# uci-cbcl/RP-Net

Hardware: AMD Instinct MI355X
Metric: support/query pairs/sec (fwd+bwd, 1-shot 256x256, T=5) (higher is better)
Workload: dtype f32

## Files before the change

rpnet_amd/csrc/conv_wgrad.hip:

```cpp
#include <algorithm>
#include <stdlib.h>

#include "common.h"

namespace rpnet {

template <int WM, int WN>
__global__ __launch_bounds__(256) void conv_wgrad_kernel(const rpnet_conv_desc d, const float* __restrict__ dy,
                                                          float* __restrict__ partial, const int M, const int Cin,
                                                          const int Cout, const int tiles_n, const int steps_per_split) {
    constexpr int BM = 64 * WM, BN = 64 * WN, BK = 32;
    constexpr int A_F4 = BM / 32, B_F4 = BN / 32;
    constexpr int A_RW = BM / 4, B_RW = BN / 4;
    __shared__ __attribute__((aligned(16))) float smem[BK * BM + BK * BN];
    float* As = smem;
    float* Bs = smem + BK * BM;

    const int t = threadIdx.x;
    const int lane = t & 63, wv = t >> 6;
    const int li = lane & 31, h = lane >> 5;
    const int wm = wv >> 1, wn = wv & 1;
    const int tm = blockIdx.x / tiles_n, tn = blockIdx.x - tm * tiles_n;
    const int cm0 = tm * BM, n0 = tn * BN;
    const int tap = blockIdx.y;
// ... 112 lines not shown
    const int li = lane & 31, h = lane >> 5;
    const int wm = wv >> 1, wn = wv & 1;
    int tile, z;
    if ((ksplit & 7) == 0) {
        const int xcd = blockIdx.x & 7, j = blockIdx.x >> 3;
        z = (j / tiles) * 8 + xcd;
        tile = j - (j / tiles) * tiles;
    } else {
        z = blockIdx.x / tiles;
        tile = blockIdx.x - z * tiles;
    }
    const int tm = tile / tiles_n, tn = tile - tm * tiles_n;
    const int cm0 = tm * BM, n0 = tn * BN;

    const int H = d.H, W = d.W, HW = H * W;
    const int ups = d.upsample;
    const int Hs = H >> ups, Ws = W >> ups;
    const float* src; int Cs, cc;
    if (cm0 < d.C0) { src = d.x0; Cs = d.C0; cc = cm0; } else { src = d.x1; Cs = d.C1; cc = cm0 - d.C0; }

    const int total_steps = (M + BK - 1) / BK;
    const int s_begin = z * steps_per_split;
    const int s_end = min(s_begin + steps_per_split, total_steps);

    const __amdgpu_buffer_rsrc_t rsx = __builtin_amdgcn_make_buffer_rsrc(
        const_cast<float*>(src), (short)0, (int)((size_t)d.N * Hs * Ws * Cs * 4), 0x00020000);
    const __amdgpu_buffer_rsrc_t rsy = __builtin_amdgcn_make_buffer_rsrc(
        const_cast<float*>(dy), (short)0, (int)((size_t)M * Cout * 4), 0x00020000);
    const int cs4 = Cs * 4;
    int qoff[A_IT], kyv[A_IT], c16[A_IT];
#pragma unroll
    for (int i = 0; i < A_IT; ++i) {
        const int e = t + 256 * i;
        const int r = e >> 4;
        const int kyi = r / SJ, j = r - kyi * SJ;
        kyv[i] = kyi - 1;
        qoff[i] = j - 1 + (kyi - 1) * W;
        c16[i] = (e & 15) * 16;
    }
    f32x4 ra[A_IT], rb[2];
    auto load_tile = [&](int st) {
        const int p0 = st * BK;
#pragma unroll
        for (int i = 0; i < A_IT; ++i) {
            const int q = p0 + qoff[i];
            int pix, yq;
            if (POW2) {
                yq = (q >> lw) & (H - 1);
                pix = ups ? (((q >> (lw + lh)) * Hs + (yq >> 1)) * Ws + ((q & (W - 1)) >> 1)) : q;
            } else {
                const int n = q / HW, rem = q - n * HW;
                yq = rem / W;
                const int xq = rem - yq * W;
                pix = (n * Hs + (yq >> ups)) * Ws + (xq >> ups);
            }
            const int yp = yq - kyv[i];
            const bool ok = (unsigned)q < (unsigned)M && (unsigned)yp < (unsigned)H;
            const int voff = ok ? pix * cs4 + c16[i] : (int)0x80000000;
            ra[i] = __builtin_bit_cast(f32x4, __builtin_amdgcn_raw_buffer_load_b128(rsx, voff, cc * 4, 0));
            if (INSCALE) {
                const float sv = d.in_scale[ok ? pix : 0];
                ra[i] *= d.in_scale_mode == 2 ? 1.f - sv : sv;
            }
        }
#pragma unroll
        for (int i = 0; i < 2; ++i) {
            const int e = t + 256 * i;
            rb[i] = __builtin_bit_cast(f32x4, __builtin_amdgcn_raw_buffer_load_b128(rsy, (p0 + (e >> 4)) * Cout * 4 + (e & 15) * 16, n0 * 4, 0));
        }
    };
    auto store_tile = [&](int st) {
        float* As = smem;
        float* Bs = smem + A_SZ;
#pragma unroll
        for (int i = 0; i < A_IT; ++i) {
            const int e = t + 256 * i;
            if (e < 3 * SJ * (BM / 4)) *reinterpret_cast<f32x4*>(&As[e * 4]) = ra[i];
        }
#pragma unroll
        for (int i = 0; i < 2; ++i) {
            const int e = t + 256 * i;
            const int p = st * BK + (e >> 4);
            const int ox = POW2 ? (p & (W - 1)) : (p % W);
            *reinterpret_cast<f32x4*>(&Bs[e * 4]) = rb[i] * (ox >= 1 ? 1.f : 0.f);
            *reinterpret_cast<f32x4*>(&Bs[B_SZ + e * 4]) = rb[i];
            *reinterpret_cast<f32x4*>(&Bs[2 * B_SZ + e * 4]) = rb[i] * (ox <= W - 2 ? 1.f : 0.f);
        }
    };

    f32x16 acc[9];
#pragma unroll
    for (int a = 0; a < 9; ++a)
#pragma unroll
        for (int r = 0; r < 16; ++r) acc[a][r] = 0.f;

    if (s_begin < s_end) {
        load_tile(s_begin);
        store_tile(s_begin);
        __syncthreads();
        const float* ap = smem + wm * 32 + li + h * BM;
        const float* bp = smem + A_SZ + wn * 32 + li + h * BN;
        for (int st = s_begin; st < s_end; ++st) {
            const bool more = st + 1 < s_end;
            if (more) load_tile(st + 1);
#pragma unroll
            for (int kp = 0; kp < BK / 2; ++kp) {
                const float bm = bp[kp * 2 * BN], b0 = bp[B_SZ + kp * 2 * BN], b1 = bp[2 * B_SZ + kp * 2 * BN];
#pragma unroll
                for (int ky = 0; ky < 3; ++ky) {
                    const float am = ap[(ky * SJ + kp * 2) * BM];
                    const float a0 = ap[(ky * SJ + kp * 2 + 1) * BM];
                    const float a1 = ap[(ky * SJ + kp * 2 + 2) * BM];
                    acc[ky * 3 + 0] = __builtin_amdgcn_mfma_f32_32x32x2f32(am, bm, acc[ky * 3 + 0], 0, 0, 0);
                    acc[ky * 3 + 1] = __builtin_amdgcn_mfma_f32_32x32x2f32(a0, b0, acc[ky * 3 + 1], 0, 0, 0);
                    acc[ky * 3 + 2] = __builtin_amdgcn_mfma_f32_32x32x2f32(a1, b1, acc[ky * 3 + 2], 0, 0, 0);
                }
            }
            __syncthreads();
            if (more) store_tile(st + 1);
            __syncthreads();
        }
    }
    if (z >= ksplit) return;
    const int col = n0 + wn * 32 + li;
#pragma unroll
    for (int tap = 0; tap < 9; ++tap) {
        float* out = partial + ((size_t)(z * 9 + tap) * Cin) * Cout;
#pragma unroll
        for (int r = 0; r < 16; ++r) {
            const int row = cm0 + wm * 32 + (r & 3) + 8 * (r >> 2) + 4 * h;
            out[(size_t)row * Cout + col] = acc[tap][r];
        }
    }
}

static int ilog2_exact(int v) {
    int l = 0;
    while ((1 << l) < v) ++l;
    return (1 << l) == v ? l : -1;
}

void wgrad9_plan(int M, int Cin, int Cout, int* ksplit, int* steps_per_split, int target_blocks) {
    const int tiles = (Cin / 64) * (Cout / 64);
    const int total_steps = (M + 31) / 32;
    long ks = tiles >= target_blocks ? 1 : (target_blocks + tiles - 1) / tiles;
    ks = std::min<long>(ks, std::max(1, total_steps / 8));
    if (ks >= 8) ks = (ks / 8) * 8;
    *steps_per_split = (int)((total_steps + ks - 1) / ks);
    int k2 = (total_steps + *steps_per_split - 1) / *steps_per_split;
    if (ks >= 8) k2 = ((k2 + 7) / 8) * 8;
    *ksplit = k2;
}

__global__ __launch_bounds__(256) void wgrad_reduce_kernel(const float* __restrict__ partial, float* __restrict__ dw,
                                                            int ksplit, int taps, int Cin_g, int Cout, int cin_w,
                                                            int off0, int split, int off1, int accumulate,
                                                            const float* __restrict__ sx, const float* __restrict__ sdy,
                                                            const float* __restrict__ sx1 = nullptr, const int c0_rows = 0) {
    __shared__ float tile[9][32][33];
    const int t = threadIdx.x;
    const int ci0 = blockIdx.x * 32, co0 = blockIdx.y * 32;
    const size_t zstride = (size_t)taps * Cin_g * Cout;
    const int tap_lo = gridDim.z > 1 ? blockIdx.z : 0, tap_hi = gridDim.z > 1 ? blockIdx.z + 1 : taps;
    const int rr = t >> 3, c4 = (t & 7) * 4;
    const int cin = ci0 + rr;
    const bool ok = cin < cin_w;
    const int row = ok ? (cin < split ? off0 + cin : off1 + (cin - split)) : 0;
    const float scl = sx ? ((sx1 && row >= c0_rows) ? *sx1 : *sx) * *sdy : 1.f;
    auto sum_tap = [&](int tap) -> f32x4 {
        f32x4 s0 = {0.f, 0.f, 0.f, 0.f}, s1 = s0, s2 = s0, s3 = s0;
        if (ok) {
            const float* p = partial + ((size_t)tap * Cin_g + row) * Cout + co0 + c4;
            int z = 0;
            for (; z + 4 <= ksplit; z += 4) {
                s0 += *reinterpret_cast<const f32x4*>(p + (size_t)z * zstride);
                s1 += *reinterpret_cast<const f32x4*>(p + (size_t)(z + 1) * zstride);
                s2 += *reinterpret_cast<const f32x4*>(p + (size_t)(z + 2) * zstride);
                s3 += *reinterpret_cast<const f32x4*>(p + (size_t)(z + 3) * zstride);
            }
            for (; z < ksplit; ++z) s0 += *reinterpret_cast<const f32x4*>(p + (size_t)z * zstride);
        }
        f32x4 s = (s0 + s1) + (s2 + s3);
        if (sx) s *= scl;
        return s;
    };
    auto put = [&](int tap, const f32x4 s) {
#pragma unroll
        for (int k = 0; k < 4; ++k) tile[tap][rr][c4 + k] = s[k];
    };
    int tap = tap_lo;
    for (; tap + 3 <= tap_hi; tap += 3) {
        const f32x4 a0 = sum_tap(tap), a1 = sum_tap(tap + 1), a2 = sum_tap(tap + 2);
        put(tap, a0); put(tap + 1, a1); put(tap + 2, a2);
    }
    for (; tap < tap_hi; ++tap) put(tap, sum_tap(tap));
    __syncthreads();
    const int ncin = min(32, cin_w - ci0);
    if (gridDim.z > 1) {
        for (int e = t; e < 32 * ncin; e += 256) {
            const int col = e / ncin, c = e - col * ncin;
            float* o = dw + ((size_t)(co0 + col) * cin_w + ci0 + c) * taps + tap_lo;
            *o = accumulate ? *o + tile[tap_lo][c][col] : tile[tap_lo][c][col];
        }
        return;
    }
    const int rowlen = ncin * taps;
    for (int e = t; e < 32 * rowlen; e += 256) {
        const int col = e / rowlen, r = e - col * rowlen;
        const int c = r / taps, tap = r - c * taps;
        float* o = dw + ((size_t)(co0 + col) * cin_w + ci0) * taps + r;
        *o = accumulate ? *o + tile[tap][c][col] : tile[tap][c][col];
    }
}

static dim3 reduce_grid(int cin_w, int Cout, int taps) {
    const int tx = cdiv(cin_w, 32), ty = Cout / 32;
    return dim3(tx, ty, (long)tx * ty >= 256 ? 1 : taps);
}

__global__ __launch_bounds__(256) void pack_weight_kernel(const float* __restrict__ w, float* __restrict__ wp,
                                                           float* __restrict__ wd, int taps, int Cin_g, int Cout,
                                                           int cin_w, int off0, int split, int off1) {
    __shared__ float tile[9][32][33];
    const int t = threadIdx.x;
    const int ci0 = blockIdx.x * 32, co0 = blockIdx.y * 32;
    const int ncin = min(32, cin_w - ci0);
    const int nel = ncin * taps;
    for (int e = t; e < 32 * nel; e += 256) {
        const int col = e / nel, r = e - col * nel;
        const int c = r / taps, tap = r - c * taps;
        tile[tap][c][col] = w[((size_t)(co0 + col) * cin_w + ci0) * taps + r];
    }
    __syncthreads();
    for (int e = t; e < taps * 32 * 32; e += 256) {
        const int cl = e & 31, c = (e >> 5) & 31, tap = e >> 10;
        if (c < ncin) {
            const int cin = ci0 + c;
            const int row = cin < split ? off0 + cin : off1 + (cin - split);
            wp[(((size_t)tap * (Cin_g >> 2) + (row >> 2)) * Cout + co0 + cl) * 4 + (row & 3)] = tile[tap][c][cl];
        }
    }
    if (wd) {
        for (int e = t; e < taps * 32 * 32; e += 256) {
            const int q = e & 3, c = (e >> 2) & 31, cq = (e >> 7) & 7, tap = e >> 10;
            if (c < ncin) {
                const int cin = ci0 + c;
                const int row = cin < split ? off0 + cin : off1 + (cin - split);
                const int cout = co0 + cq * 4 + q;
                const int tf = taps - 1 - tap;
                wd[(((size_t)tf * (Cout >> 2) + (cout >> 2)) * Cin_g + row) * 4 + q] = tile[tap][c][cq * 4 + q];
            }
        }
    }
}

static void wgrad_plan(int M, int Cin, int Cout, int taps, int* bm, int* bn, int* ksplit, int* steps_per_split) {
    *bm = (Cin % 128 == 0 && taps > 1) ? 128 : 64;
    *bn = (Cout % 128 == 0) ? 128 : 64;
    long tiles = (long)(Cin / *bm) * (Cout / *bn) * taps;
    if (tiles < 1) tiles = 1;
    const int total_steps = (M + 31) / 32;
    int ks = (int)((768 + tiles - 1) / tiles);
    ks = max(1, min(ks, max(1, total_steps / 8)));
    if (taps == 1) ks = min(ks, kWgrad1MaxSplits);
    *steps_per_split = (total_steps + ks - 1) / ks;
    if (taps == 9) *steps_per_split += *steps_per_split & 1;
    *ksplit = (total_steps + *steps_per_split - 1) / *steps_per_split;
}

int conv_wgrad9_split(const rpnet_conv_desc* d, const void* dy, float* part9, int M, int Cin, int Cout, int ks9, int sps9,
                      hipStream_t s);
bool conv_wgrad9_dma_one_plane_ok(const rpnet_conv_desc* d, int M, int sps9);
int conv_wgrad9_split_dma(const rpnet_conv_desc* d, const void* dy, float* part9, int M, int Cin, int Cout, int ks9, int sps9,
                          hipStream_t s);
bool conv_wgrad9_ring_ok(const rpnet_conv_desc* d, int M, int sps9);
int conv_wgrad9_ring(const rpnet_conv_desc* d, const void* dy, float* part9, int M, int Cin, int Cout, int ks9, int sps9, hipStream_t s);
void wgrad1_split_plan(int M, int Cin, int Cout, int* ksplit, int* steps_per_split);
int conv_wgrad1_split(const rpnet_conv_desc* d, const void* dy, float* part, int M, int Cin, int Cout, int ks, int sps, hipStream_t s);

}

extern "C" size_t rpnet_conv_wgrad_workspace_bytes(int N, int H, int W, int cin_gathered, int cout, int taps) {
    int bm, bn, ks, sps;
    rpnet::wgrad_plan(N * H * W, cin_gathered, cout, taps, &bm, &bn, &ks, &sps);
    size_t need = (size_t)ks * taps * cin_gathered * cout * sizeof(float);
    if (taps == 9 && cin_gathered % 64 == 0 && cout % 64 == 0) {
        int ks9, sps9;
        rpnet::wgrad9_plan(N * H * W, cin_gathered, cout, &ks9, &sps9, 512);
        need = std::max(need, (size_t)ks9 * 9 * cin_gathered * cout * sizeof(float));
    }
    return need;
}

extern "C" int rpnet_conv_wgrad(const rpnet_conv_desc* d, const float* dy, float* dw, int cin_w, int cin_off0,
                                int cin_split, int cin_off1, void* workspace, size_t workspace_bytes,
                                rpnet_stream_t stream) {
    using namespace rpnet;
    RPNET_REQUIRE(d && d->x0 && workspace && (dy || dw), RPNET_ERR_ARG, "conv_wgrad: null pointer");
    RPNET_REQUIRE((dy && dw) || (d->split_planes && d->dilation <= 1), RPNET_ERR_ARG,
                  "conv_wgrad: the two-phase form (dy or dw NULL) exists for the split kernels only");
    const int Cin = d->C0 + d->C1, Cout = d->Co0 + d->Co1;
    RPNET_REQUIRE(d->taps == 9 || d->taps == 1, RPNET_ERR_ARG, "conv_wgrad: taps must be 9 or 1");
    RPNET_REQUIRE(!d->split_planes || d->dilation <= 1, RPNET_ERR_ARG,
                  "conv_wgrad: split operands are implemented for dense 3x3 and 1x1 taps only");
    RPNET_REQUIRE(Cin % 64 == 0 && Cout % 64 == 0, RPNET_ERR_SHAPE, "conv_wgrad: Cin %d / Cout %d not multiples of 64", Cin, Cout);
    RPNET_REQUIRE((long)d->N * d->H * d->W < (1L << 31), RPNET_ERR_SHAPE, "conv_wgrad: too many pixels");
    const int M = d->N * d->H * d->W;
    RPNET_REQUIRE((size_t)M * (d->C0 > d->C1 ? d->C0 : d->C1) * 4 < (1UL << 31) && (size_t)M * Cout * 4 < (1UL << 31),
                  RPNET_ERR_SHAPE, "conv_wgrad: an operand exceeds the 2 GiB buffer-descriptor range (split the batch)");
    hipStream_t s = (hipStream_t)stream;
    if (d->taps == 9 && d->dilation <= 1) {
        RPNET_REQUIRE(d->C1 == 0 || d->C0 % 64 == 0, RPNET_ERR_SHAPE, "conv_wgrad: source split %d not aligned to 64", d->C0);
        int ks9, sps9;
        wgrad9_plan(M, Cin, Cout, &ks9, &sps9, d->split_planes ? 256 : 512);
        const size_t need9 = (size_t)ks9 * 9 * Cin * Cout * sizeof(float);
        RPNET_REQUIRE(workspace_bytes >= need9, RPNET_ERR_WORKSPACE, "conv_wgrad: workspace %zu < %zu", workspace_bytes, need9);
        const int tiles_n9 = Cout / 64, tiles9 = (Cin / 64) * tiles_n9;
        const int lw = ilog2_exact(d->W), lh = ilog2_exact(d->H);
        float* part9 = (float*)workspace;
        if (d->split_planes) {
            RPNET_REQUIRE(d->split_planes >= 1 && d->split_planes <= 3 && d->in_scale_mode == 0, RPNET_ERR_ARG,
                          "conv_wgrad: split operands take 1 to 3 planes and no in_scale");
            if (dy) {
                const int tv = d->tune & 255;
                const bool dma = (d->split_planes == 2 || conv_wgrad9_dma_one_plane_ok(d, M, sps9)) && tv != 8 && tv != 4;
                const bool ring = dma && tv != 16 && conv_wgrad9_ring_ok(d, M, sps9);
                if (int rc = ring ? conv_wgrad9_ring(d, dy, part9, M, Cin, Cout, ks9, sps9, s)
                             : dma ? conv_wgrad9_split_dma(d, dy, part9, M, Cin, Cout, ks9, sps9, s)
                                   : conv_wgrad9_split(d, dy, part9, M, Cin, Cout, ks9, sps9, s))
                    return rc;
            }
            if (!dw) return RPNET_OK;
            RPNET_REQUIRE(d->split_planes == 3 || (d->acc_scale_x && d->acc_scale_dy), RPNET_ERR_ARG,
                          "conv_wgrad: fp16 planes need acc_scale_x and acc_scale_dy");
            hipLaunchKernelGGL(wgrad_reduce_kernel, reduce_grid(cin_w, Cout, 9), dim3(256), 0, s, part9, dw, ks9, 9, Cin,
                               Cout, cin_w, cin_off0, cin_split, cin_off1, d->accumulate,
                               d->split_planes <= 2 ? d->acc_scale_x : nullptr, d->acc_scale_dy);
            return check_launch("wgrad_reduce");
        }
#define RPNET_W9(P2, IS, LW, LH)                                                                                   \
    hipLaunchKernelGGL((conv_wgrad9_kernel<P2, IS>), dim3(tiles9 * ks9), dim3(256), 0, s, *d, dy, part9, M, Cin, Cout, \
                       tiles9, tiles_n9, ks9, sps9, LW, LH)
        const bool p2 = lw >= 0 && lh >= 0, is = d->in_scale_mode != 0;
        if (p2 && is) RPNET_W9(true, true, lw, lh);
        else if (p2) RPNET_W9(true, false, lw, lh);
        else if (is) RPNET_W9(false, true, 0, 0);
        else RPNET_W9(false, false, 0, 0);
#undef RPNET_W9
        int rc9 = check_launch("conv_wgrad9");
        if (rc9) return rc9;
        hipLaunchKernelGGL(wgrad_reduce_kernel, reduce_grid(cin_w, Cout, 9), dim3(256), 0, s, part9, dw, ks9, 9, Cin,
                           Cout, cin_w, cin_off0, cin_split, cin_off1, d->accumulate, (const float*)nullptr, (const float*)nullptr);
        return check_launch("wgrad_reduce");
    }
    if (d->split_planes && d->taps == 1) {
        RPNET_REQUIRE(d->split_planes >= 1 && d->split_planes <= 3 && d->in_scale_mode == 0 && d->upsample == 0, RPNET_ERR_ARG,
                      "conv_wgrad: split 1x1 operands take 1 to 3 planes, no in_scale, no upsampling");
        RPNET_REQUIRE(d->C1 == 0 || (d->C0 % 64 == 0 && d->x1), RPNET_ERR_SHAPE, "conv_wgrad: source split %d not aligned to 64", d->C0);
        int ks1, sps1;
        wgrad1_split_plan(M, Cin, Cout, &ks1, &sps1);
        const size_t need1 = (size_t)ks1 * Cin * Cout * sizeof(float);
        RPNET_REQUIRE(workspace_bytes >= need1, RPNET_ERR_WORKSPACE, "conv_wgrad: workspace %zu < %zu", workspace_bytes, need1);
        float* part1 = (float*)workspace;
        if (dy)
            if (int rc = conv_wgrad1_split(d, dy, part1, M, Cin, Cout, ks1, sps1, s)) return rc;
        if (!dw) return RPNET_OK;
        RPNET_REQUIRE(d->split_planes == 3 || (d->acc_scale_x && d->acc_scale_dy), RPNET_ERR_ARG,
                      "conv_wgrad: fp16 planes need acc_scale_x and acc_scale_dy");
        hipLaunchKernelGGL(wgrad_reduce_kernel, reduce_grid(cin_w, Cout, 1), dim3(256), 0, s, part1, dw, ks1, 1, Cin, Cout, cin_w,
                           cin_off0, cin_split, cin_off1, d->accumulate, d->split_planes <= 2 ? d->acc_scale_x : nullptr,
                           d->acc_scale_dy, d->split_planes <= 2 ? d->acc_scale_x1 : nullptr, d->C0);
        return check_launch("wgrad_reduce");
    }
    int bm, bn, ks, sps;
    wgrad_plan(M, Cin, Cout, d->taps, &bm, &bn, &ks, &sps);
    RPNET_REQUIRE(d->C1 == 0 || d->C0 % bm == 0, RPNET_ERR_SHAPE, "conv_wgrad: source split %d not aligned to tile %d", d->C0, bm);
    const size_t need = (size_t)ks * d->taps * Cin * Cout * sizeof(float);
    RPNET_REQUIRE(workspace_bytes >= need, RPNET_ERR_WORKSPACE, "conv_wgrad: workspace %zu < %zu", workspace_bytes, need);
    const int tiles_n = Cout / bn, tiles = (Cin / bm) * tiles_n;
    dim3 grid(tiles, d->taps, ks);
    float* part = (float*)workspace;
    if (bm == 128 && bn == 128)
        hipLaunchKernelGGL((conv_wgrad_kernel<2, 2>), grid, dim3(256), 0, s, *d, dy, part, M, Cin, Cout, tiles_n, sps);
    else if (bm == 128)
        hipLaunchKernelGGL((conv_wgrad_kernel<2, 1>), grid, dim3(256), 0, s, *d, dy, part, M, Cin, Cout, tiles_n, sps);
    else if (bn == 128)
        hipLaunchKernelGGL((conv_wgrad_kernel<1, 2>), grid, dim3(256), 0, s, *d, dy, part, M, Cin, Cout, tiles_n, sps);
    else
        hipLaunchKernelGGL((conv_wgrad_kernel<1, 1>), grid, dim3(256), 0, s, *d, dy, part, M, Cin, Cout, tiles_n, sps);
    int rc = check_launch("conv_wgrad");
    if (rc) return rc;
    hipLaunchKernelGGL(wgrad_reduce_kernel, reduce_grid(cin_w, Cout, d->taps), dim3(256), 0, s, part, dw, ks, d->taps,
                       Cin, Cout, cin_w, cin_off0, cin_split, cin_off1, d->accumulate, (const float*)nullptr, (const float*)nullptr);
    return check_launch("wgrad_reduce");
}

extern "C" int rpnet_pack_conv_weight(const float* w, float* wp, float* wd, int cout, int cin, int taps, int cin_off0,
                                      int cin_split, int cin_off1, int cin_pad, rpnet_stream_t stream) {
    using namespace rpnet;
    RPNET_REQUIRE(w && wp, RPNET_ERR_ARG, "pack_conv_weight: null pointer");
    RPNET_REQUIRE(cout > 0 && cout % 32 == 0 && cin_pad % 4 == 0 && (taps == 9 || taps == 1), RPNET_ERR_SHAPE,
                  "pack_conv_weight: cout %d cin_pad %d taps %d", cout, cin_pad, taps);
    RPNET_REQUIRE(cin > 0 && cin_split >= 0 && cin_split <= cin && cin_off0 >= 0 && cin_off1 >= 0, RPNET_ERR_SHAPE,
                  "pack_conv_weight: cin %d cin_split %d cin_off0 %d cin_off1 %d", cin, cin_split, cin_off0, cin_off1);
    RPNET_REQUIRE((long)cin_off0 + cin_split <= cin_pad && (long)cin_off1 + (cin - cin_split) <= cin_pad, RPNET_ERR_SHAPE,
                  "pack_conv_weight: channel ranges exceed cin_pad");
    RPNET_REQUIRE(pack_ranges_disjoint(cin, cin_off0, cin_split, cin_off1), RPNET_ERR_SHAPE, "pack_conv_weight: channel ranges overlap");
    hipLaunchKernelGGL(pack_weight_kernel, dim3(cdiv(cin, 32), cout / 32), dim3(256), 0, (hipStream_t)stream, w, wp, wd,
                       taps, cin_pad, cout, cin, cin_off0, cin_split, cin_off1);
    return check_launch("pack_conv_weight");
}
```

rpnet_amd/csrc/conv_wgrad_up4.hip:

```cpp
#include <type_traits>

#include "common.h"
#include "lds_dma.h"
#include "split_bf16.h"

namespace rpnet {

using s16x4u = __attribute__((ext_vector_type(4))) short;
typedef __attribute__((address_space(3))) s16x4u lds_s16x4u_t;

template <int N, int I = 0, typename F>
__device__ __forceinline__ void static_for_wu(F&& f) {
    if constexpr (I < N) {
        f(std::integral_constant<int, I>{});
        static_for_wu<N, I + 1>(f);
    }
}

template <bool K64>
__global__ __launch_bounds__(256, 1) void conv_wgrad_up4_kernel(const rpnet_conv_desc d, const unsigned short* __restrict__ dy,
                                                                 float* __restrict__ partial, const int Ml, const int Cin, const int Cout,
                                                                 const int tiles, const int tiles_n, const int ksplit,
                                                                 const int steps_per_split, const int lw, const int lh) {
    constexpr int NP = 2, BK = 32, RB = 128;
// ... 112 lines not shown
    const int cbyte = (16 * (g & 1) + 4 * (L & 3)) * 2;
    const int a_off = krow * RB + (((wm ^ ((krow >> 1) & 1)) << 6) | cbyte);
    const unsigned char* const aptr = smem + a_off;
    int b_off[2];
#pragma unroll
    for (int kxl = 0; kxl < 2; ++kxl) {
        const int r = krow + 2 - (px + kxl);
        b_off[kxl] = BOFF + r * RB + (((wn ^ ((r >> 1) & 1)) << 6) | cbyte);
    }
    const int b_zero = BOFF + ZROW * RB + ((wn << 6) | cbyte);
    auto tr = [&](const unsigned char* p) -> s16x4u { return __builtin_amdgcn_ds_read_tr16_b64_v4i16((lds_s16x4u_t*)p); };

    s16x4u afr[2][2][NP][2], bfr[2][2][NP][2];
    constexpr int NSL = K64 ? 2 : 1;
    const unsigned char* bsel[2][2][NSL][2];
    const unsigned char* bconst[2][2][2];
#pragma unroll
    for (int s2 = 0; s2 < 2; ++s2)
#pragma unroll
        for (int kxl = 0; kxl < 2; ++kxl)
#pragma unroll
            for (int e = 0; e < 2; ++e) {
                bconst[s2][kxl][e] = smem + b_off[kxl] + (16 * s2 + 4 * e) * RB;
#pragma unroll
                for (int sl = 0; sl < NSL; ++sl) bsel[s2][kxl][sl][e] = bconst[s2][kxl][e];
            }
    const unsigned char* const bzero = smem + b_zero;
    auto b_addr = [&](auto sc, const int st) {
        constexpr int s = decltype(sc)::value;
#pragma unroll
        for (int sl = 0; sl < NSL; ++sl)
#pragma unroll
            for (int e = 0; e < 2; ++e) {
                const int q = st * PXS + BK * sl + 16 * s + 4 * e + krow;
                const int ox = q & (Wl - 1);
                bsel[s][0][sl][e] = (px != 0 || ox <= Wl - 2) ? bconst[s][0][e] : bzero;
                bsel[s][1][sl][e] = (px == 0 || ox >= 1) ? bconst[s][1][e] : bzero;
            }
    };
    constexpr int NR = NP * 8, NMMA = (K64 ? 2 : nprod<NP>()) * 4;
    static_assert(NR <= 2 * NMMA, "at most two fragment reads behind each MFMA");
    auto read_frag = [&](auto sc, auto kc, auto stagec) {
        constexpr int s = decltype(sc)::value, k = decltype(kc)::value, stage = decltype(stagec)::value;
        constexpr int grp = k / 8, r = (k - grp * 8) >> 1, e = k & 1;
        constexpr int pa = K64 ? grp : NP - 1 - grp, pb = grp;
        if constexpr (r == 0 || r == 3) {
            constexpr int kyl = r == 0 ? 0 : 1;
            constexpr int off = stage * A_STAGE + pa * A_PLANE + (kyl * BK + 16 * s + 4 * e) * RB;
            afr[s][kyl][pa][e] = tr(aptr + off);
        } else {
            constexpr int kxl = r - 1;
            bfr[s][kxl][pb][e] = tr(bsel[s][kxl][K64 ? pb : 0][e] + (stage * B_STAGE + pb * B_PLANE));
        }
    };
    auto frag = [](const s16x4u lo, const s16x4u hi) {
        return __builtin_bit_cast(bf16x8, __builtin_shufflevector(lo, hi, 0, 1, 2, 3, 4, 5, 6, 7));
    };
    auto mma_one = [&](auto sc, auto mc) {
        constexpr int s = decltype(sc)::value, m = decltype(mc)::value;
        constexpr int q = m / 4, tap = m - q * 4, kyl = tap >> 1, kxl = tap & 1;
        constexpr int pa = K64 ? q : prod_a<NP>(q), pb = K64 ? q : prod_b<NP>(q);
        acc[tap] = mma16<NP>(frag(afr[s][kyl][pa][0], afr[s][kyl][pa][1]), frag(bfr[s][kxl][pb][0], bfr[s][kxl][pb][1]), acc[tap]);
    };
    using I0 = std::integral_constant<int, 0>;
    using I1 = std::integral_constant<int, 1>;

    if (s_begin < s_end) {
        auto stc = [&](int st) { return st < s_end ? st : s_end - 1; };
        dma_step(std::integral_constant<int, 0>{}, s_begin);
        dma_step(std::integral_constant<int, 1>{}, stc(s_begin + 1));
        dma_step(std::integral_constant<int, 2>{}, stc(s_begin + 2));
        wait_all_but_one_step();
        __builtin_amdgcn_s_barrier();
        b_addr(I0{}, s_begin);
        static_for_wu<NR>([&](auto kc) { read_frag(I0{}, kc, I0{}); });
        auto step = [&](auto kc4, const int st) {
            constexpr int K = decltype(kc4)::value;
            using SK = std::integral_constant<int, K>;
            using SN = std::integral_constant<int, (K + 1) & 3>;
            using SD = std::integral_constant<int, (K + 3) & 3>;
            const int dst_step = stc(st + 3);
            b_addr(I1{}, st);
            __builtin_amdgcn_sched_barrier(0);
            static_for_wu<NMMA>([&](auto mc) {
                constexpr int m = decltype(mc)::value;
                mma_one(I0{}, mc);
                __builtin_amdgcn_sched_barrier(0);
                read_frag(I1{}, mc, SK{});
                __builtin_amdgcn_sched_barrier(0);
                if constexpr (m < NR - NMMA) {
                    read_frag(I1{}, std::integral_constant<int, NMMA + m>{}, SK{});
                    __builtin_amdgcn_sched_barrier(0);
                }
                if constexpr (m == NMMA / 2 - 1 || m == NMMA - 3) {
                    dma_x(std::integral_constant<int, (m == NMMA / 2 - 1 ? 0 : 1)>{}, SD{}, dst_step);
                    __builtin_amdgcn_sched_barrier(0);
                }
            });
            b_addr(I0{}, st + 1);
            __builtin_amdgcn_sched_barrier(0);
            static_for_wu<NMMA>([&](auto mc) {
                constexpr int m = decltype(mc)::value;
                mma_one(I1{}, mc);
                __builtin_amdgcn_sched_barrier(0);
                read_frag(I0{}, mc, SN{});
                __builtin_amdgcn_sched_barrier(0);
                if constexpr (m < NR - NMMA) {
                    read_frag(I0{}, std::integral_constant<int, NMMA + m>{}, SN{});
                    __builtin_amdgcn_sched_barrier(0);
                }
                if constexpr (m == NMMA / 2 - 1) {
                    dma_y(SD{}, false, dst_step);
                    __builtin_amdgcn_sched_barrier(0);
                }
                if constexpr (m == NMMA - 3) {
                    if (wv == 0) dma_y(SD{}, true, dst_step);
                    __builtin_amdgcn_sched_barrier(0);
                }
            });
            wait_all_but_one_step();
            __builtin_amdgcn_s_barrier();
        };
        for (int st = s_begin; st < s_end; st += 4) {
            step(std::integral_constant<int, 0>{}, st);
            if (st + 1 >= s_end) break;
            step(std::integral_constant<int, 1>{}, st + 1);
            if (st + 2 >= s_end) break;
            step(std::integral_constant<int, 2>{}, st + 2);
            if (st + 3 >= s_end) break;
            step(std::integral_constant<int, 3>{}, st + 3);
        }
        asm volatile("s_waitcnt vmcnt(0)" ::: "memory");
        __builtin_amdgcn_s_barrier();
    }
    if (z >= ksplit) return;
    const int li = lane & 31, h = lane >> 5;
    constexpr int SW = 36;
    float* slab = reinterpret_cast<float*>(smem) + wv * 32 * SW;
#pragma unroll
    for (int tap = 0; tap < 4; ++tap) {
#pragma unroll
        for (int r = 0; r < 16; ++r) slab[((r & 3) + 8 * (r >> 2) + 4 * h) * SW + li] = acc[tap][r];
        __builtin_amdgcn_wave_barrier();
        float* out = partial + ((size_t)((phase * ksplit + z) * 4 + tap) * Cin + cm0 + wm * 32) * Cout + n0 + wn * 32;
#pragma unroll
        for (int q = 0; q < 4; ++q) {
            const int gidx = q * 64 + lane, rr = gidx >> 3, c4 = gidx & 7;
            *reinterpret_cast<f32x4*>(out + (size_t)rr * Cout + c4 * 4) = *reinterpret_cast<const f32x4*>(&slab[rr * SW + c4 * 4]);
        }
        __builtin_amdgcn_wave_barrier();
    }
}

__global__ __launch_bounds__(256) void wgrad_up4_reduce_kernel(const float* __restrict__ partial, float* __restrict__ dw, const int ksplit,
                                                                const int Cin, const int Cout, const int accumulate,
                                                                const float* __restrict__ sx, const float* __restrict__ sdy) {
    __shared__ float tile[9][32][33];
    const int t = threadIdx.x;
    const int ci0 = blockIdx.x * 32, co0 = blockIdx.y * 32;
    const int rr = t >> 3, c4 = (t & 7) * 4;
    const size_t tstride = (size_t)Cin * Cout, zstride = 4 * tstride, pstride = (size_t)ksplit * zstride;
    const float scl = *sx * *sdy;
    f32x4 v[4][4];
#pragma unroll
    for (int ph = 0; ph < 4; ++ph)
#pragma unroll
        for (int sl = 0; sl < 4; ++sl) {
            const float* p = partial + ph * pstride + sl * tstride + (size_t)(ci0 + rr) * Cout + co0 + c4;
            f32x4 s0 = {0.f, 0.f, 0.f, 0.f}, s1 = s0;
            int z = 0;
            for (; z + 2 <= ksplit; z += 2) {
                s0 += *reinterpret_cast<const f32x4*>(p + (size_t)z * zstride);
                s1 += *reinterpret_cast<const f32x4*>(p + (size_t)(z + 1) * zstride);
            }
            if (z < ksplit) s0 += *reinterpret_cast<const f32x4*>(p + (size_t)z * zstride);
            v[ph][sl] = s0 + s1;
        }
#pragma unroll
    for (int ky = 0; ky < 3; ++ky)
#pragma unroll
        for (int kx = 0; kx < 3; ++kx) {
            f32x4 s = {0.f, 0.f, 0.f, 0.f};
#pragma unroll
            for (int ph = 0; ph < 4; ++ph) {
                const int py = ph >> 1, px = ph & 1;
                const int r = py == 0 ? (ky >= 1) : (ky >= 2), c = px == 0 ? (kx >= 1) : (kx >= 2);
                s += v[ph][r * 2 + c];
            }
            s *= scl;
#pragma unroll
            for (int k = 0; k < 4; ++k) tile[ky * 3 + kx][rr][c4 + k] = s[k];
        }
    __syncthreads();
    const int rowlen = 32 * 9;
    for (int e = t; e < 32 * rowlen; e += 256) {
        const int col = e / rowlen, r = e - col * rowlen;
        const int c = r / 9, tap = r - c * 9;
        float* o = dw + ((size_t)(co0 + col) * Cin + ci0) * 9 + r;
        *o = accumulate ? *o + tile[tap][c][col] : tile[tap][c][col];
    }
}

static int ilog2u(int v) {
    int l = 0;
    while ((1 << l) < v) ++l;
    return (1 << l) == v ? l : -1;
}

static void up4_wgrad_plan(int Ml, int Cin, int Cout, int pxs, int* ksplit, int* sps) {
    const int tiles = (Cin / 64) * (Cout / 64) * 4;
    const int total_steps = (Ml + pxs - 1) / pxs;
    long ks = tiles >= 256 ? 1 : (256 + tiles - 1) / tiles;
    ks = std::min<long>(ks, std::max(1, total_steps / 8));
    if (ks >= 8) ks = (ks / 8) * 8;
    *sps = (int)((total_steps + ks - 1) / ks);
    int k2 = (total_steps + *sps - 1) / *sps;
    if (ks >= 8) k2 = ((k2 + 7) / 8) * 8;
    *ksplit = k2;
}

static bool up4_wgrad_ok(const rpnet_conv_desc* d) {
    if (!d || (d->split_planes != 2 && d->split_planes != 1) || d->C1 || d->Co1 || d->x1 || d->H % 2 || d->W % 2) return false;
    const int Hl = d->H / 2, Wl = d->W / 2;
    if (ilog2u(Wl) < 3 || ilog2u(Hl) < 0 || d->C0 % 64 || d->Co0 % 64) return false;
    const size_t lim = (size_t)1 << 31;
    return (size_t)d->N * Hl * Wl * d->C0 * 4 < lim && (size_t)d->N * d->H * d->W * d->Co0 * 4 < lim &&
           ((size_t)d->N * Hl * Wl) % (d->split_planes == 1 ? 64 : 32) == 0;
}

}

extern "C" int rpnet_conv_wgrad_up4_supported(const rpnet_conv_desc* d) { return rpnet::up4_wgrad_ok(d) ? 1 : 0; }

extern "C" size_t rpnet_conv_wgrad_up4_workspace_bytes(int N, int H, int W, int cin, int cout) {
    int ks, sps, ks1, sps1;
    rpnet::up4_wgrad_plan(N * (H / 2) * (W / 2), cin, cout, 32, &ks, &sps);
    rpnet::up4_wgrad_plan(N * (H / 2) * (W / 2), cin, cout, 64, &ks1, &sps1);
    return (size_t)4 * (ks > ks1 ? ks : ks1) * 4 * cin * cout * sizeof(float);
}

extern "C" int rpnet_conv_wgrad_up4(const rpnet_conv_desc* d, const void* dy, float* dw, void* workspace, size_t workspace_bytes,
                                    rpnet_stream_t stream) {
    using namespace rpnet;
    RPNET_REQUIRE(d && d->x0 && workspace && (dy || dw), RPNET_ERR_ARG, "conv_wgrad_up4: null pointer");
    RPNET_REQUIRE(up4_wgrad_ok(d), RPNET_ERR_SHAPE, "conv_wgrad_up4: N=%d H=%d W=%d C0=%d Co0=%d planes=%d do not fit (rpnet_conv_wgrad_up4_supported)",
                  d->N, d->H, d->W, d->C0, d->Co0, d->split_planes);
    const int Hl = d->H / 2, Wl = d->W / 2, Ml = d->N * Hl * Wl, Cin = d->C0, Cout = d->Co0;
    int ks, sps;
    const bool one = d->split_planes == 1;
    up4_wgrad_plan(Ml, Cin, Cout, one ? 64 : 32, &ks, &sps);
    RPNET_REQUIRE(workspace_bytes >= rpnet_conv_wgrad_up4_workspace_bytes(d->N, d->H, d->W, Cin, Cout), RPNET_ERR_WORKSPACE, "conv_wgrad_up4: workspace");
    hipStream_t s = (hipStream_t)stream;
    float* part = (float*)workspace;
    if (dy) {
        const int tiles_n = Cout / 64, tiles = (Cin / 64) * tiles_n;
        if (one)
            hipLaunchKernelGGL(conv_wgrad_up4_kernel<true>, dim3(tiles * ks * 4), dim3(256), 0, s, *d, (const unsigned short*)dy, part, Ml, Cin, Cout,
                               tiles, tiles_n, ks, sps, ilog2u(Wl), ilog2u(Hl));
        else
            hipLaunchKernelGGL(conv_wgrad_up4_kernel<false>, dim3(tiles * ks * 4), dim3(256), 0, s, *d, (const unsigned short*)dy, part, Ml, Cin, Cout,
                               tiles, tiles_n, ks, sps, ilog2u(Wl), ilog2u(Hl));
        if (int rc = check_launch("conv_wgrad_up4")) return rc;
    }
    if (!dw) return RPNET_OK;
    RPNET_REQUIRE(d->acc_scale_x && d->acc_scale_dy, RPNET_ERR_ARG, "conv_wgrad_up4: fp16 planes need acc_scale_x and acc_scale_dy");
    hipLaunchKernelGGL(wgrad_up4_reduce_kernel, dim3(Cin / 32, Cout / 32), dim3(256), 0, s, (const float*)part, dw, ks, Cin, Cout, d->accumulate,
                       d->acc_scale_x, d->acc_scale_dy);
    return check_launch("wgrad_up4_reduce");
}
```

Measured before the change: 510.4.

## Split wgrad split-K reductions across waves with fewer channels per block

```diff
diff --git a/include/rpnet_wgrad_reduce_abi.h b/include/rpnet_wgrad_reduce_abi.h
--- /dev/null
+++ b/include/rpnet_wgrad_reduce_abi.h
@@ -0,0 +1,18 @@
+#ifndef RPNET_WGRAD_REDUCE_ABI_H
+#define RPNET_WGRAD_REDUCE_ABI_H
+
+#ifdef __cplusplus
+extern "C" {
+#endif
+
+int rpnet_wgrad_reduce(const float* partial, float* dw, int ksplit, int taps, int cin_g, int cout, int cin_w, int cin_off0,
+                       int cin_split, int cin_off1, int accumulate, const float* sx, const float* sdy, const float* sx1,
+                       int c0_rows, void* stream);
+
+int rpnet_wgrad_up4_reduce(const float* partial, float* dw, int ksplit, int cin, int cout, int accumulate, const float* sx,
+                           const float* sdy, void* stream);
+
+#ifdef __cplusplus
+}
+#endif
+#endif
diff --git a/rpnet_amd/csrc/conv_wgrad.hip b/rpnet_amd/csrc/conv_wgrad.hip
--- a/rpnet_amd/csrc/conv_wgrad.hip
+++ b/rpnet_amd/csrc/conv_wgrad.hip
@@ -288,70 +288,122 @@
     *ksplit = k2;
 }
 
-__global__ __launch_bounds__(256) void wgrad_reduce_kernel(const float* __restrict__ partial, float* __restrict__ dw,
-                                                            int ksplit, int taps, int Cin_g, int Cout, int cin_w,
-                                                            int off0, int split, int off1, int accumulate,
-                                                            const float* __restrict__ sx, const float* __restrict__ sdy,
-                                                            const float* __restrict__ sx1 = nullptr, const int c0_rows = 0) {
-    __shared__ float tile[9][32][33];
+
+template <int NT, int ZB>
+__device__ __forceinline__ void reduce_walk(const float* __restrict__ p, const unsigned voff, const size_t tstride, const size_t stride,
+                                            const int count, f32x4 (&s)[NT]) {
+    int k = 0;
+    for (; k + ZB <= count; k += ZB, p += ZB * stride) {
+        f32x4 v[ZB][NT];
+#pragma unroll
+        for (int b = 0; b < ZB; ++b)
+#pragma unroll
+            for (int j = 0; j < NT; ++j) v[b][j] = *reinterpret_cast<const f32x4*>(p + b * stride + j * tstride + voff);
+#pragma unroll
+        for (int b = 0; b < ZB; ++b)
+#pragma unroll
+            for (int j = 0; j < NT; ++j) s[j] += v[b][j];
+    }
+    for (; k < count; ++k, p += stride)
+#pragma unroll
+        for (int j = 0; j < NT; ++j) s[j] += *reinterpret_cast<const f32x4*>(p + j * tstride + voff);
+}
+
+template <int NT, int ZB>
+__device__ __forceinline__ void reduce_chain(const float* __restrict__ p, const unsigned voff, const size_t tstride, const size_t zstride,
+                                             const int q, const int ksplit, f32x4 (&s)[NT]) {
+    const int n = ksplit >> 2;
+#pragma unroll
+    for (int j = 0; j < NT; ++j) s[j] = f32x4{0.f, 0.f, 0.f, 0.f};
+    reduce_walk<NT, ZB>(p + q * zstride, voff, tstride, 4 * zstride, n, s);
+    if (q == 0) reduce_walk<NT, ZB>(p + (size_t)(4 * n) * zstride, voff, tstride, zstride, ksplit - 4 * n, s);
+}
+
+template <int ZC, int TPB>
+__global__ __launch_bounds__(256) __attribute__((amdgpu_waves_per_eu(TPB == 9 ? 4 : 8, 8))) void wgrad_reduce_kernel(
+    const float* __restrict__ partial, float* __restrict__ dw, const int ksplit, const int taps, const int Cin_g, const int Cout,
+    const int cin_w, const int off0, const int split, const int off1, const int accumulate, const float* __restrict__ sx,
+    const float* __restrict__ sdy, const float* __restrict__ sx1, const int c0_rows) {
+#pragma clang fp contract(off)
+    RPNET_PASS_PRIORITY();
+    static_assert(ZC == 1 || ZC == 4, "chains per thread: all four or one");
+    constexpr int CT = 32 / ZC;
+    constexpr int NT = TPB % 3 == 0 ? 3 : 1;
+    constexpr int ZB = NT == 3 ? 2 : 8;
+    constexpr int QS = CT * TPB * 33;
+    __shared__ float tile[ZC * QS];
+    __shared__ float rscl[CT];
     const int t = threadIdx.x;
-    const int ci0 = blockIdx.x * 32, co0 = blockIdx.y * 32;
-    const size_t zstride = (size_t)taps * Cin_g * Cout;
-    const int tap_lo = gridDim.z > 1 ? blockIdx.z : 0, tap_hi = gridDim.z > 1 ? blockIdx.z + 1 : taps;
-    const int rr = t >> 3, c4 = (t & 7) * 4;
-    const int cin = ci0 + rr;
-    const bool ok = cin < cin_w;
-    const int row = ok ? (cin < split ? off0 + cin : off1 + (cin - split)) : 0;
-    const float scl = sx ? ((sx1 && row >= c0_rows) ? *sx1 : *sx) * *sdy : 1.f;
-    auto sum_tap = [&](int tap) -> f32x4 {
-        f32x4 s0 = {0.f, 0.f, 0.f, 0.f}, s1 = s0, s2 = s0, s3 = s0;
-        if (ok) {
-            const float* p = partial + ((size_t)tap * Cin_g + row) * Cout + co0 + c4;
-            int z = 0;
-            for (; z + 4 <= ksplit; z += 4) {
-                s0 += *reinterpret_cast<const f32x4*>(p + (size_t)z * zstride);
-                s1 += *reinterpret_cast<const f32x4*>(p + (size_t)(z + 1) * zstride);
-                s2 += *reinterpret_cast<const f32x4*>(p + (size_t)(z + 2) * zstride);
-                s3 += *reinterpret_cast<const f32x4*>(p + (size_t)(z + 3) * zstride);
-            }
-            for (; z < ksplit; ++z) s0 += *reinterpret_cast<const f32x4*>(p + (size_t)z * zstride);
-        }
-        f32x4 s = (s0 + s1) + (s2 + s3);
-        if (sx) s *= scl;
-        return s;
+    const int ci0 = blockIdx.x * CT, co0 = blockIdx.y * 32, tap0 = blockIdx.z * TPB;
+    const int q = ZC == 4 ? uni(t >> 6) : 0, rr = (t >> 3) & (CT - 1), c4 = (t & 7) * 4;
+    auto gathered = [&](const int cin) { return cin < split ? off0 + cin : off1 + (cin - split); };
+    if (t < CT && ci0 + t < cin_w) rscl[t] = sx ? ((sx1 && gathered(ci0 + t) >= c0_rows) ? *sx1 : *sx) * *sdy : 1.f;
+    if (ci0 + rr < cin_w) {
+        const size_t tstride = (size_t)Cin_g * Cout, zstride = (size_t)taps * tstride;
+        const float* p = partial + (size_t)tap0 * tstride;
+        const unsigned voff = (unsigned)gathered(ci0 + rr) * Cout + co0 + c4;
+        float* lt = tile + (q * CT + rr) * TPB * 33 + c4;
+        const f32x4 zero = {0.f, 0.f, 0.f, 0.f};
+#pragma unroll 1
+        for (int tg = 0; tg < TPB; tg += NT) {
+            f32x4 s[NT];
+            reduce_chain<NT, ZB>(p + tg * tstride, voff, tstride, zstride, q, ksplit, s);
+#pragma unroll
+            for (int j = 0; j < NT; ++j) {
+                if (ZC == 1) s[j] = (s[j] + zero) + (zero + zero);
+#pragma unroll
+                for (int k = 0; k < 4; ++k) lt[(tg + j) * 33 + k] = s[j][k];
+            }
+        }
+    }
+    __syncthreads();
+    const int ncin = min(CT, cin_w - ci0);
+    auto emit = [&](const int rowlen) {
+#pragma unroll 1
+        for (int e = t; e < 32 * rowlen; e += 256) {
+            const int col = e / rowlen, r = e - col * rowlen;
+            const int c = r / TPB;
+            const float* l = tile + r * 33 + col;
+            float v = ZC == 4 ? (l[0] + l[QS]) + (l[2 * QS] + l[3 * QS]) : l[0];
+            v *= rscl[c];
+            float* o = dw + ((size_t)(co0 + col) * cin_w + ci0 + c) * taps + tap0 + (r - c * TPB);
+            *o = accumulate ? *o + v : v;
+        }
     };
-    auto put = [&](int tap, const f32x4 s) {
-#pragma unroll
-        for (int k = 0; k < 4; ++k) tile[tap][rr][c4 + k] = s[k];
-    };
-    int tap = tap_lo;
-    for (; tap + 3 <= tap_hi; tap += 3) {
-        const f32x4 a0 = sum_tap(tap), a1 = sum_tap(tap + 1), a2 = sum_tap(tap + 2);
-        put(tap, a0); put(tap + 1, a1); put(tap + 2, a2);
-    }
-    for (; tap < tap_hi; ++tap) put(tap, sum_tap(tap));
-    __syncthreads();
-    const int ncin = min(32, cin_w - ci0);
-    if (gridDim.z > 1) {
-        for (int e = t; e < 32 * ncin; e += 256) {
-            const int col = e / ncin, c = e - col * ncin;
-            float* o = dw + ((size_t)(co0 + col) * cin_w + ci0 + c) * taps + tap_lo;
-            *o = accumulate ? *o + tile[tap_lo][c][col] : tile[tap_lo][c][col];
-        }
-        return;
-    }
-    const int rowlen = ncin * taps;
-    for (int e = t; e < 32 * rowlen; e += 256) {
-        const int col = e / rowlen, r = e - col * rowlen;
-        const int c = r / taps, tap = r - c * taps;
-        float* o = dw + ((size_t)(co0 + col) * cin_w + ci0) * taps + r;
-        *o = accumulate ? *o + tile[tap][c][col] : tile[tap][c][col];
-    }
-}
-
-static dim3 reduce_grid(int cin_w, int Cout, int taps) {
-    const int tx = cdiv(cin_w, 32), ty = Cout / 32;
-    return dim3(tx, ty, (long)tx * ty >= 256 ? 1 : taps);
+    if (ncin == CT) emit(CT * TPB);
+    else emit(ncin * TPB);
+}
+
+struct ReduceCut { int zc, tpb; };
+static ReduceCut wgrad_reduce_cut(int cin_w, int Cout, int taps, int ksplit) {
+    ReduceCut c;
+    c.zc = ksplit >= 4 ? 4 : 1;
+    c.tpb = 1;
+    if (taps == 9) {
+        const long tiles = (long)cdiv(cin_w, 32 / c.zc) * (Cout / 32);
+        c.tpb = tiles >= 768 ? 9 : 3 * tiles >= 768 ? 3 : 1;
+    }
+    return c;
+}
+
+int launch_wgrad_reduce(const float* partial, float* dw, int ksplit, int taps, int Cin_g, int Cout, int cin_w, int off0, int split,
+                        int off1, int accumulate, const float* sx, const float* sdy, const float* sx1, int c0_rows, hipStream_t s) {
+    const ReduceCut c = wgrad_reduce_cut(cin_w, Cout, taps, ksplit);
+    const dim3 grid(cdiv(cin_w, 32 / c.zc), Cout / 32, taps / c.tpb);
+#define RPNET_RED(ZC, TPB)                                                                                                     \
+    hipLaunchKernelGGL((wgrad_reduce_kernel<ZC, TPB>), grid, dim3(256), 0, s, partial, dw, ksplit, taps, Cin_g, Cout, cin_w, off0, \
+                       split, off1, accumulate, sx, sdy, sx1, c0_rows)
+    if (c.zc == 4) {
+        if (c.tpb == 9) RPNET_RED(4, 9);
+        else if (c.tpb == 3) RPNET_RED(4, 3);
+        else RPNET_RED(4, 1);
+    } else {
+        if (c.tpb == 9) RPNET_RED(1, 9);
+        else if (c.tpb == 3) RPNET_RED(1, 3);
+        else RPNET_RED(1, 1);
+    }
+#undef RPNET_RED
+    return check_launch("wgrad_reduce");
 }
 
 __global__ __launch_bounds__(256) void pack_weight_kernel(const float* __restrict__ w, float* __restrict__ wp,
@@ -469,10 +521,8 @@
             if (!dw) return RPNET_OK;
             RPNET_REQUIRE(d->split_planes == 3 || (d->acc_scale_x && d->acc_scale_dy), RPNET_ERR_ARG,
                           "conv_wgrad: fp16 planes need acc_scale_x and acc_scale_dy");
-            hipLaunchKernelGGL(wgrad_reduce_kernel, reduce_grid(cin_w, Cout, 9), dim3(256), 0, s, part9, dw, ks9, 9, Cin,
-                               Cout, cin_w, cin_off0, cin_split, cin_off1, d->accumulate,
-                               d->split_planes <= 2 ? d->acc_scale_x : nullptr, d->acc_scale_dy);
-            return check_launch("wgrad_reduce");
+            return launch_wgrad_reduce(part9, dw, ks9, 9, Cin, Cout, cin_w, cin_off0, cin_split, cin_off1, d->accumulate,
+                                       d->split_planes <= 2 ? d->acc_scale_x : nullptr, d->acc_scale_dy, nullptr, 0, s);
         }
 #define RPNET_W9(P2, IS, LW, LH)                                                                                   \
     hipLaunchKernelGGL((conv_wgrad9_kernel<P2, IS>), dim3(tiles9 * ks9), dim3(256), 0, s, *d, dy, part9, M, Cin, Cout, \
@@ -485,9 +535,8 @@
 #undef RPNET_W9
         int rc9 = check_launch("conv_wgrad9");
         if (rc9) return rc9;
-        hipLaunchKernelGGL(wgrad_reduce_kernel, reduce_grid(cin_w, Cout, 9), dim3(256), 0, s, part9, dw, ks9, 9, Cin,
-                           Cout, cin_w, cin_off0, cin_split, cin_off1, d->accumulate, (const float*)nullptr, (const float*)nullptr);
-        return check_launch("wgrad_reduce");
+        return launch_wgrad_reduce(part9, dw, ks9, 9, Cin, Cout, cin_w, cin_off0, cin_split, cin_off1, d->accumulate, nullptr, nullptr,
+                                   nullptr, 0, s);
     }
     if (d->split_planes && d->taps == 1) {
         RPNET_REQUIRE(d->split_planes >= 1 && d->split_planes <= 3 && d->in_scale_mode == 0 && d->upsample == 0, RPNET_ERR_ARG,
@@ -503,10 +552,9 @@
         if (!dw) return RPNET_OK;
         RPNET_REQUIRE(d->split_planes == 3 || (d->acc_scale_x && d->acc_scale_dy), RPNET_ERR_ARG,
                       "conv_wgrad: fp16 planes need acc_scale_x and acc_scale_dy");
-        hipLaunchKernelGGL(wgrad_reduce_kernel, reduce_grid(cin_w, Cout, 1), dim3(256), 0, s, part1, dw, ks1, 1, Cin, Cout, cin_w,
-                           cin_off0, cin_split, cin_off1, d->accumulate, d->split_planes <= 2 ? d->acc_scale_x : nullptr,
-                           d->acc_scale_dy, d->split_planes <= 2 ? d->acc_scale_x1 : nullptr, d->C0);
-        return check_launch("wgrad_reduce");
+        return launch_wgrad_reduce(part1, dw, ks1, 1, Cin, Cout, cin_w, cin_off0, cin_split, cin_off1, d->accumulate,
+                                   d->split_planes <= 2 ? d->acc_scale_x : nullptr, d->acc_scale_dy,
+                                   d->split_planes <= 2 ? d->acc_scale_x1 : nullptr, d->C0, s);
     }
     int bm, bn, ks, sps;
     wgrad_plan(M, Cin, Cout, d->taps, &bm, &bn, &ks, &sps);
@@ -526,9 +574,8 @@
         hipLaunchKernelGGL((conv_wgrad_kernel<1, 1>), grid, dim3(256), 0, s, *d, dy, part, M, Cin, Cout, tiles_n, sps);
     int rc = check_launch("conv_wgrad");
     if (rc) return rc;
-    hipLaunchKernelGGL(wgrad_reduce_kernel, reduce_grid(cin_w, Cout, d->taps), dim3(256), 0, s, part, dw, ks, d->taps,
-                       Cin, Cout, cin_w, cin_off0, cin_split, cin_off1, d->accumulate, (const float*)nullptr, (const float*)nullptr);
-    return check_launch("wgrad_reduce");
+    return launch_wgrad_reduce(part, dw, ks, d->taps, Cin, Cout, cin_w, cin_off0, cin_split, cin_off1, d->accumulate, nullptr, nullptr,
+                               nullptr, 0, s);
 }
 
 extern "C" int rpnet_pack_conv_weight(const float* w, float* wp, float* wd, int cout, int cin, int taps, int cin_off0,
@@ -546,3 +593,20 @@
                        taps, cin_pad, cout, cin, cin_off0, cin_split, cin_off1);
     return check_launch("pack_conv_weight");
 }
+
+#include "rpnet_wgrad_reduce_abi.h"
+
+extern "C" int rpnet_wgrad_reduce(const float* partial, float* dw, int ksplit, int taps, int cin_g, int cout, int cin_w, int cin_off0,
+                                  int cin_split, int cin_off1, int accumulate, const float* sx, const float* sdy, const float* sx1,
+                                  int c0_rows, void* stream) {
+    using namespace rpnet;
+    RPNET_REQUIRE(partial && dw && (!sx || sdy), RPNET_ERR_ARG, "wgrad_reduce: null pointer");
+    RPNET_REQUIRE(ksplit >= 1 && (taps == 9 || taps == 1) && cout > 0 && cout % 32 == 0 && cin_w >= 1 && cin_g >= 1, RPNET_ERR_SHAPE,
+                  "wgrad_reduce: ksplit %d taps %d cin_g %d cout %d cin_w %d", ksplit, taps, cin_g, cout, cin_w);
+    RPNET_REQUIRE(cin_split >= 0 && cin_split <= cin_w && cin_off0 >= 0 && cin_off1 >= 0 && (long)cin_off0 + cin_split <= cin_g &&
+                      (long)cin_off1 + (cin_w - cin_split) <= cin_g,
+                  RPNET_ERR_SHAPE, "wgrad_reduce: channel ranges exceed cin_g %d", cin_g);
+    RPNET_REQUIRE(cdiv(cin_w, 8) <= 65535 && cout / 32 <= 65535, RPNET_ERR_SHAPE, "wgrad_reduce: too many tiles");
+    return launch_wgrad_reduce(partial, dw, ksplit, taps, cin_g, cout, cin_w, cin_off0, cin_split, cin_off1, accumulate, sx, sdy, sx1,
+                               c0_rows, (hipStream_t)stream);
+}
diff --git a/rpnet_amd/csrc/conv_wgrad_up4.hip b/rpnet_amd/csrc/conv_wgrad_up4.hip
--- a/rpnet_amd/csrc/conv_wgrad_up4.hip
+++ b/rpnet_amd/csrc/conv_wgrad_up4.hip
@@ -288,53 +288,66 @@
     }
 }
 
-__global__ __launch_bounds__(256) void wgrad_up4_reduce_kernel(const float* __restrict__ partial, float* __restrict__ dw, const int ksplit,
-                                                                const int Cin, const int Cout, const int accumulate,
-                                                                const float* __restrict__ sx, const float* __restrict__ sdy) {
-    __shared__ float tile[9][32][33];
+__global__ __launch_bounds__(256) __attribute__((amdgpu_waves_per_eu(8, 8))) void wgrad_up4_reduce_kernel(
+    const float* __restrict__ partial, float* __restrict__ dw, const int ksplit, const int Cin, const int Cout, const int accumulate,
+    const float* __restrict__ sx, const float* __restrict__ sdy) {
+#pragma clang fp contract(off)
+    RPNET_PASS_PRIORITY();
+    constexpr int CT = 8;
+    __shared__ float tile[16 * CT * 33];
     const int t = threadIdx.x;
-    const int ci0 = blockIdx.x * 32, co0 = blockIdx.y * 32;
-    const int rr = t >> 3, c4 = (t & 7) * 4;
+    const int ci0 = blockIdx.x * CT, co0 = blockIdx.y * 32;
+    const int ph = uni(t >> 6), rr = (t >> 3) & (CT - 1), c4 = (t & 7) * 4;
     const size_t tstride = (size_t)Cin * Cout, zstride = 4 * tstride, pstride = (size_t)ksplit * zstride;
     const float scl = *sx * *sdy;
-    f32x4 v[4][4];
-#pragma unroll
-    for (int ph = 0; ph < 4; ++ph)
-#pragma unroll
-        for (int sl = 0; sl < 4; ++sl) {
-            const float* p = partial + ph * pstride + sl * tstride + (size_t)(ci0 + rr) * Cout + co0 + c4;
-            f32x4 s0 = {0.f, 0.f, 0.f, 0.f}, s1 = s0;
-            int z = 0;
-            for (; z + 2 <= ksplit; z += 2) {
-                s0 += *reinterpret_cast<const f32x4*>(p + (size_t)z * zstride);
-                s1 += *reinterpret_cast<const f32x4*>(p + (size_t)(z + 1) * zstride);
-            }
-            if (z < ksplit) s0 += *reinterpret_cast<const f32x4*>(p + (size_t)z * zstride);
-            v[ph][sl] = s0 + s1;
-        }
-#pragma unroll
-    for (int ky = 0; ky < 3; ++ky)
-#pragma unroll
-        for (int kx = 0; kx < 3; ++kx) {
-            f32x4 s = {0.f, 0.f, 0.f, 0.f};
-#pragma unroll
-            for (int ph = 0; ph < 4; ++ph) {
-                const int py = ph >> 1, px = ph & 1;
-                const int r = py == 0 ? (ky >= 1) : (ky >= 2), c = px == 0 ? (kx >= 1) : (kx >= 2);
-                s += v[ph][r * 2 + c];
-            }
-            s *= scl;
-#pragma unroll
-            for (int k = 0; k < 4; ++k) tile[ky * 3 + kx][rr][c4 + k] = s[k];
-        }
+    const float* p = partial + ph * pstride;
+    const unsigned voff = (unsigned)(ci0 + rr) * Cout + co0 + c4;
+#pragma unroll
+    for (int sp = 0; sp < 4; sp += 2) {
+        const float* p0 = p + sp * tstride;
+        const float* p1 = p0 + tstride;
+        f32x4 a0 = {0.f, 0.f, 0.f, 0.f}, a1 = a0, b0 = a0, b1 = a0;
+        int z = 0;
+        for (; z + 2 <= ksplit; z += 2) {
+            const f32x4 va0 = *reinterpret_cast<const f32x4*>(p0 + (size_t)z * zstride + voff);
+            const f32x4 va1 = *reinterpret_cast<const f32x4*>(p0 + (size_t)(z + 1) * zstride + voff);
+            const f32x4 vb0 = *reinterpret_cast<const f32x4*>(p1 + (size_t)z * zstride + voff);
+            const f32x4 vb1 = *reinterpret_cast<const f32x4*>(p1 + (size_t)(z + 1) * zstride + voff);
+            a0 += va0; a1 += va1; b0 += vb0; b1 += vb1;
+        }
+        if (z < ksplit) {
+            const f32x4 va0 = *reinterpret_cast<const f32x4*>(p0 + (size_t)z * zstride + voff);
+            const f32x4 vb0 = *reinterpret_cast<const f32x4*>(p1 + (size_t)z * zstride + voff);
+            a0 += va0; b0 += vb0;
+        }
+        const f32x4 va = a0 + a1, vb = b0 + b1;
+        float* l = tile + ((ph * 4 + sp) * CT + rr) * 33 + c4;
+#pragma unroll
+        for (int k = 0; k < 4; ++k) { l[k] = va[k]; l[CT * 33 + k] = vb[k]; }
+    }
     __syncthreads();
-    const int rowlen = 32 * 9;
+    constexpr int rowlen = CT * 9;
     for (int e = t; e < 32 * rowlen; e += 256) {
         const int col = e / rowlen, r = e - col * rowlen;
         const int c = r / 9, tap = r - c * 9;
+        const int ky = tap / 3, kx = tap - ky * 3;
+        float s = 0.f;
+#pragma unroll
+        for (int f = 0; f < 4; ++f) {
+            const int py = f >> 1, px = f & 1;
+            const int sr = py == 0 ? (ky >= 1) : (ky >= 2), sc = px == 0 ? (kx >= 1) : (kx >= 2);
+            s += tile[((f * 4 + sr * 2 + sc) * CT + c) * 33 + col];
+        }
+        s *= scl;
         float* o = dw + ((size_t)(co0 + col) * Cin + ci0) * 9 + r;
-        *o = accumulate ? *o + tile[tap][c][col] : tile[tap][c][col];
-    }
+        *o = accumulate ? *o + s : s;
+    }
+}
+
+int launch_wgrad_up4_reduce(const float* partial, float* dw, int ksplit, int Cin, int Cout, int accumulate, const float* sx,
+                            const float* sdy, hipStream_t s) {
+    hipLaunchKernelGGL(wgrad_up4_reduce_kernel, dim3(Cin / 8, Cout / 32), dim3(256), 0, s, partial, dw, ksplit, Cin, Cout, accumulate, sx, sdy);
+    return check_launch("wgrad_up4_reduce");
 }
 
 static int ilog2u(int v) {
@@ -400,7 +413,16 @@
     }
     if (!dw) return RPNET_OK;
     RPNET_REQUIRE(d->acc_scale_x && d->acc_scale_dy, RPNET_ERR_ARG, "conv_wgrad_up4: fp16 planes need acc_scale_x and acc_scale_dy");
-    hipLaunchKernelGGL(wgrad_up4_reduce_kernel, dim3(Cin / 32, Cout / 32), dim3(256), 0, s, (const float*)part, dw, ks, Cin, Cout, d->accumulate,
-                       d->acc_scale_x, d->acc_scale_dy);
-    return check_launch("wgrad_up4_reduce");
-}
+    return launch_wgrad_up4_reduce(part, dw, ks, Cin, Cout, d->accumulate, d->acc_scale_x, d->acc_scale_dy, s);
+}
+
+#include "rpnet_wgrad_reduce_abi.h"
+
+extern "C" int rpnet_wgrad_up4_reduce(const float* partial, float* dw, int ksplit, int cin, int cout, int accumulate, const float* sx,
+                                      const float* sdy, void* stream) {
+    using namespace rpnet;
+    RPNET_REQUIRE(partial && dw && sx && sdy, RPNET_ERR_ARG, "wgrad_up4_reduce: null pointer");
+    RPNET_REQUIRE(ksplit >= 1 && cin > 0 && cin % 8 == 0 && cout > 0 && cout % 32 == 0 && cin / 8 <= 65535 && cout / 32 <= 65535,
+                  RPNET_ERR_SHAPE, "wgrad_up4_reduce: ksplit %d cin %d cout %d", ksplit, cin, cout);
+    return launch_wgrad_up4_reduce(partial, dw, ksplit, cin, cout, accumulate, sx, sdy, (hipStream_t)stream);
+}
```

Measured after the change: 510.5, median of 2. Within noise of the previous version (+0.0%).
